# GPflow/GPflow

Hardware: AMD Instinct MI355X
Metric: svgp_elbo_steps_per_s (higher is better)
Workload: dtype f64; 1 GPU; SVGP RBF(ARD)+Gaussian ELBO, N=1e+06 M=2048 D=8 P=1 whitened, 8192 minibatch rows per GPU per step (BASELINE metric config Cm); global_batch=8192

## Files before the change

### gpflow_amd/csrc/gemm.hip

```cpp
#include "gpk_internal.h"
#include <mutex>
#include <stdlib.h>
#include <algorithm>
#include <type_traits>

namespace {

constexpr int BK = kGemmBK;
constexpr int LDSS = kGemmLDSS;
constexpr int GROUP_N = kGemmGroupN;

template <int BM, int BN, int WGM, int WGN>
struct TileCfg {
  static constexpr int WM = BM / WGM, WN = BN / WGN;
  static constexpr int TM = WM / 16, TN = WN / 16;
  static constexpr int A_CH = BM * (BK / 2) / 256;
  static constexpr int B_CH = BN * (BK / 2) / 256;
  static constexpr size_t LDS_BYTES = 2 * (size_t)(BM + BN) * LDSS * sizeof(double);
};

__device__ __forceinline__ void tile_decode(int nl, int gx, int gy, int compact, int& tile_m, int& tile_n) {
  tile_m = 0; tile_n = 0;
  if (compact) {
    int g = 0;
// ... 34 lines not shown
  const int xcd = lin & 7, local = lin >> 3;
  const int q = total >> 3, r = total & 7;
  int nl = xcd * q + (xcd < r ? xcd : r) + local;
  if (b_tri == 1 && gx > GROUP_N) nl = lin;
  tile_decode(nl, gx, gy, compact, tile_m, tile_n);
}

__device__ __forceinline__ d2 load2(const double* __restrict__ base, long ld, int row, int nrows,
                                    int k, int ke, bool vec_ok) {
  d2 v = {0.0, 0.0};
  if (row < nrows && k < ke) {
    const double* ptr = base + (long)row * ld + k;
    if (vec_ok && k + 1 < ke) {
      v = *reinterpret_cast<const d2*>(ptr);
    } else {
      v.x = ptr[0];
      if (k + 1 < ke) v.y = ptr[1];
    }
  }
  return v;
}

template <int BM, int BN, int WGM, int WGN>
__global__ __launch_bounds__(256, 2) void gemm_nt_kernel(GemmArgs p, int gx, int gy, int total, int compact) {
  using Cfg = TileCfg<BM, BN, WGM, WGN>;
  constexpr int WM = Cfg::WM, WN = Cfg::WN, TM = Cfg::TM, TN = Cfg::TN;
  constexpr int A_CH = Cfg::A_CH, B_CH = Cfg::B_CH;
  extern __shared__ __attribute__((aligned(16))) double smem[];
  if (p.sig_ptr && threadIdx.x == 0 && blockIdx.x == 0 && blockIdx.y == 0)
    __hip_atomic_store(p.sig_ptr, p.sig_val, __ATOMIC_RELAXED, __HIP_MEMORY_SCOPE_SYSTEM);

  const int tid = threadIdx.x, lane = tid & 63, wave = tid >> 6;
  const int wm = wave / WGN, wn = wave % WGN;
  const int bz = p.k_off_step ? (int)gridDim.y - 1 - (int)blockIdx.y : (int)blockIdx.y;

  int tile_m, tile_n;
  if (BM == 64 && BN == 64 && p.tail_first1 > 0) {
    int tm, tn;
    tile_decode(p.tail_first1 - 1 + ((int)blockIdx.x >> 2), gx, gy, compact, tm, tn);
    tile_m = 2 * tm + (((int)blockIdx.x >> 1) & 1);
    tile_n = 2 * tn + ((int)blockIdx.x & 1);
  } else if (p.tile_snake) {
    const int r = (int)blockIdx.x >> 8, c = (int)blockIdx.x & 255, R = (int)gridDim.x >> 8;
    const int rr = (r & 1) ? R - 1 - (r >> 1) : (r >> 1);
    if (p.tile_snake == 2) {
      const int xcd = c & 7, s = c >> 3, rpx = gy >> 3;
      const int q = rr * 32 + (((r ^ bz) & 1) ? 31 - s : s);
      tile_n = q / rpx;
      tile_m = xcd * rpx + (q - tile_n * rpx);
    } else {
      const int nl = rr * 256 + ((r & 1) ? 255 - c : c);
      if (nl >= total) return;
      tile_n = nl / gy;
      tile_m = nl - tile_n * gy;
    }
  } else {
    tile_order(blockIdx.x, p.b_tri, gx, gy, total, compact, tile_m, tile_n);
  }
  const int m0 = tile_m * BM, n0 = tile_n * BN;
  if (p.c_lower && n0 > m0 + BM - 1) return;
  if (m0 >= p.m || n0 >= p.n) return;

  const double* __restrict__ A = p.A + (long)bz * p.strideA;
  const double* __restrict__ B = p.B + (long)bz * p.strideB;

  int kb = 0, ke = p.k;
  const int koff = bz * p.k_off_step;
  if (p.b_tri && (n0 + BN < p.n ? n0 + BN : p.n) <= p.b_tri_rows) {
    if (p.b_tri == 1) {
      int f = n0 + p.b_tri_off - koff;
      kb = (f > 0 ? f : 0) & ~(BK - 1);
    } else {
      int l = n0 + BN + p.b_tri_off - koff;
      ke = l < p.k ? l : p.k;
    }
  }
  if (p.a_tri == 1) {
    int f = m0 - koff;
    f = (f > 0 ? f : 0) & ~(BK - 1);
    kb = kb > f ? kb : f;
  } else if (p.a_tri == 2) {
// ... 158 lines not shown
        } else {
          if ((lane & 15) == 0) smem[wn * BM + (row - m0)] = s;
        }
      }
    if constexpr (WN < 64) {
      constexpr int WPS = 64 / WN;
      __syncthreads();
      if (wn % WPS == 0 && (lane & 15) == 0) {
#pragma unroll
        for (int i = 0; i < TM; ++i)
#pragma unroll
          for (int r = 0; r < 4; ++r) {
            const int row = row_base + i * 16 + 4 * r;
            double s = smem[wn * BM + (row - m0)];
#pragma unroll
            for (int u = 1; u < WPS; ++u) s += smem[(wn + u) * BM + (row - m0)];
            if (row < p.m) part[(long)(tile_n * (BN / 64) + (wn * WN) / 64) * p.part_ld + row] = s;
          }
      }
    }
  }
}


__global__ __launch_bounds__(256, 2) void gemm_nt_pre64(GemmArgs p, int gx, int gy, int total, int compact) {
  constexpr int BM = 64, BN = 64, MAXS = 8;
  constexpr int BUF = (BM + BN) * LDSS;
  extern __shared__ __attribute__((aligned(16))) double smem[];
  if (p.sig_ptr && threadIdx.x == 0 && blockIdx.x == 0 && blockIdx.y == 0)
    __hip_atomic_store(p.sig_ptr, p.sig_val, __ATOMIC_RELAXED, __HIP_MEMORY_SCOPE_SYSTEM);

  const int tid = threadIdx.x, lane = tid & 63, wave = tid >> 6;
  const int bz = blockIdx.y;
  int tile_m, tile_n;
  tile_order(blockIdx.x, 0, gx, gy, total, compact, tile_m, tile_n);
  const int m0 = tile_m * BM, n0 = tile_n * BN;
  if (p.c_lower && n0 > m0 + BM - 1) return;
  if (m0 >= p.m || n0 >= p.n) return;
  const double* __restrict__ A = p.A + (long)bz * p.strideA;
  const double* __restrict__ B = p.B + (long)bz * p.strideB;
  double* __restrict__ C = p.C + (long)bz * p.strideC;
  const int nkt = p.k / BK;

  d2 ra[MAXS][2], rb[MAXS][2];
  const double* pa[2];
  const double* pb[2];
// ... 581 lines not shown
      }
      return GPK_E_UNSUPPORTED;
    default: break;
  }
  constexpr int FAST = (int)kGemmFastLds, WHOLE = 160 * 1024;
  if (p.queue) {
    unsigned qbase = 0;
    GPK_TRY(queue_slot(p.queue_fetches, &b.queue, &qbase));
    b.queue_base = (int)qbase;
    return launch_tiled<gemm_nt_fast<0, false, true>, FAST>(s, grid, p.lds_bytes, b, p, p.total);
  }
  int rc = GPK_E_UNSUPPORTED;
  switch (4 * p.epi + 2 * p.pair + p.sp) {
    case 0: rc = launch_tiled<gemm_nt_fast<0, false, false, 0>, WHOLE>(s, grid, p.lds_bytes, b, p, p.total); break;
    case 2: rc = launch_tiled<gemm_nt_fast<0, true, false, 0>, FAST>(s, grid, p.lds_bytes, b, p, p.total); break;
    case 4: rc = launch_tiled<gemm_nt_fast<1, false, false, 0>, WHOLE>(s, grid, p.lds_bytes, b, p, p.total); break;
    case 5: rc = launch_tiled<gemm_nt_fast<1, false, false, 1>, WHOLE>(s, grid, p.lds_bytes, b, p, p.total); break;
    case 6: rc = launch_tiled<gemm_nt_fast<1, true, false, 0>, FAST>(s, grid, p.lds_bytes, b, p, p.total); break;
    case 7: rc = launch_tiled<gemm_nt_fast<1, true, false, 1>, FAST>(s, grid, p.lds_bytes, b, p, p.total); break;
  }
  if (rc || p.tail_tiles == 0) return rc;
  GemmArgs t = a;
  t.tail_first1 = p.tail_first1;
  return launch_generic<64, 64, 4, 1>(s, dim3(p.tail_grid_x, 1, 1), t, p, (int)p.tail_grid_x);
}

}

int gpk_gemm_tiles_n(int n) { return gpk_cdiv(n, 128); }
bool gpk_gemm_takes_latency_kernel(const GemmArgs& a) { return make_gemm_plan(a).kernel == GemmKernel::small; }
bool gpk_gemm_fuses_row_stats(const GemmArgs& a) {
  const GemmPlan p = make_gemm_plan(a);
  return p.kernel == GemmKernel::fast && p.sp;
}

namespace {
struct ProfRec { hipEvent_t e0, e1; double flops; int kind; };
bool g_prof_on = false;
ProfRec* g_prof = nullptr;
int g_prof_n = 0, g_prof_cap = 0;

double algorithmic_flops(const GemmArgs& a) {
  const double m = a.m, n = a.n, k = a.k;
  double outs = m * n;
  if (a.c_lower) outs = (m >= n) ? n * (n + 1) / 2 + (m - n) * n : m * (m + 1) / 2;
  double kk = k;
  if (a.b_tri) {
// ... 151 lines not shown
```

### gpflow_amd/csrc/gemm_plan.h

```cpp
#pragma once
#include <stddef.h>
#include <stdint.h>
#include "gpk_tune.h"

struct GemmArgs {
  const double* A; long lda; long strideA;
  const double* B; long ldb; long strideB;
  double* C; long ldc; long strideC;
  int m, n, k;
  double alpha, beta;
  int c_lower;
  int b_tri;
  int a_tri;
  int b_tri_off;
  int b_tri_rows;
  int k_off_step;
  int epi;
  int sq_cols;
  double* part; long part_ld; long stridePart;
  double* C2; long ldc2; long strideC2; int c2_cols;
  double* stat_sumsq; double* stat_mv; const double* stat_V; int stat_P;
  int batch;
  int stagger_first;
  int stagger_ticks;
// ... 42 lines not shown
  switch (t) {
    case GemmTile::t128x128: return {128, 128, 2, 2};
    case GemmTile::t128x64: return {128, 64, 2, 2};
    case GemmTile::t64x128_1x4: return {64, 128, 1, 4};
    case GemmTile::t64x128_2x2: return {64, 128, 2, 2};
    case GemmTile::t64x64: return {64, 64, 4, 1};
    default: return {32, 64, 2, 2};
  }
}
constexpr size_t gemm_tile_lds(int bm, int bn) { return 2 * (size_t)(bm + bn) * kGemmLDSS * sizeof(double); }

struct GemmPlan {
  GemmKernel kernel = GemmKernel::none;
  GemmTile tile = GemmTile::t128x128;
  int epi = 0, pair = 0, queue = 0, sp = 0;
  int kind = 0;
  int gx = 0, gy = 0, total = 0, compact = 0;
  int ldk = 0;
  unsigned grid_x = 0, grid_y = 0, grid_z = 0;
  unsigned threads = 0;
  size_t lds_bytes = 0;
  int tile_snake = 0, stagger_first = 0, stagger_ticks = 0, pair_k_align = 0, tail_first1 = 0;
  int tail_tiles = 0;
  unsigned tail_grid_x = 0;
  unsigned queue_wgs = 0, queue_fetches = 0;
};

static inline int gemm_cdiv(int a, int b) { return (a + b - 1) / b; }
static inline int gemm_nbatch(const GemmArgs& a) { return a.batch > 0 ? a.batch : 1; }

static inline int gemm_lower_tiles(int gx, int gy) {
  int total = 0;
  for (int first = 0; first < gx; first += kGemmGroupN) {
    const int gsz = (gx - first) < kGemmGroupN ? (gx - first) : kGemmGroupN;
    const int avail = gy - first;
    if (avail <= 0) break;
    const int tr = avail < gsz ? avail : gsz;
    total += tr * (tr + 1) / 2 + (avail > gsz ? (avail - gsz) * gsz : 0);
  }
  return total;
}

static inline bool gemm_rows_16b(const GemmArgs& a) {
  if ((a.lda & 1) || (a.ldb & 1) || (a.strideA & 1) || (a.strideB & 1)) return false;
  return !((reinterpret_cast<uintptr_t>(a.A) & 15) || (reinterpret_cast<uintptr_t>(a.B) & 15));
}

// ... 144 lines not shown
                          : 0;
  }
  if (EPI == 0 && a.max_wgs > 0 && nwg < (unsigned)total && nb == 1) {
    const int kb = GPK_TUNE(CAP_EXCL_LDS_KB, 84);
    if (kb > 0 && kb <= 160 && (size_t)kb * 1024 > kGemmFastLds) p.lds_bytes = (size_t)kb * 1024;
  }
  if (EPI == 0 && tail_tiles == 0 && a.max_wgs == 0 &&
      ((a.k_off_step && GPK_TUNE(KSPLIT_QUEUE, 1)) || (a.tile_queue && (long)total * nb > 512))) {
    p.queue = 1;
    p.stagger_ticks = 0;
    const long all = (long)total * nb;
    const long qw = a.stagger_first > 0 ? 2L * a.stagger_first : GPK_TUNE(QUEUE_WGS, 512);
    p.queue_wgs = (unsigned)(all < qw ? all : qw);
    p.queue_fetches = (unsigned)all + p.queue_wgs;
    p.lds_bytes = kGemmFastLds;
    p.grid_x = p.queue_wgs; p.grid_y = 1;
    return;
  }
  p.grid_x = nwg;
  if (tail_tiles > 0) {
    p.tail_tiles = tail_tiles;
    p.tail_first1 = total_all - tail_tiles + 1;
    p.tail_grid_x = (unsigned)(4 * tail_tiles);
  }
}

static inline GemmPlan make_gemm_plan(const GemmArgs& a) {
  GemmPlan p;
  p.tile_snake = a.tile_snake; p.stagger_first = a.stagger_first; p.stagger_ticks = a.stagger_ticks;
  p.pair_k_align = a.pair_k_align;
  if (a.m <= 0 || a.n <= 0) return p;
  const auto unsupported = [&p]() { p.kernel = GemmKernel::unsupported; return p; };
  if (a.stat_sumsq && !gemm_row_stats_fusable(a)) return unsupported();
  const long tiles = (long)gemm_cdiv(a.m, 128) * gemm_cdiv(a.n, 128) * gemm_nbatch(a);
  if (a.tile64 && a.epi == 0) {
    if (GPK_TUNE(REST_PRE64, 1) && gemm_pre64_ok(a)) gemm_plan_pre64(a, p);
    else gemm_plan_generic(a, p, GemmTile::t64x64);
    return p;
  }
  if (!a.no_small && gemm_small_ok(a)) {
    gemm_plan_small(a, p);
    return p;
  }
  if (a.epi == 1 && a.beta != 0.0 && a.C && !gemm_fast_ok(a)) return unsupported();
  GemmTile tile = GemmTile::t128x128;
  if (a.epi == 0 && a.k >= GPK_TUNE(HALF_TILE_KMIN, 1024) && a.m > 64 && a.n > 64 && (a.max_wgs == 0 || a.max_wgs >= tiles) &&
      (a.c_lower ? tiles / 2 : tiles) < GPK_TUNE(HALF_TILE_BELOW, 300)) {
    tile = GemmTile::t64x128_1x4;
  } else if (gemm_proj_small_tiles(a)) {
    p.tile_snake = GPK_TUNE(PROJ_SNAKE, 1);
    if (gemm_cdiv(a.n, 64) != 2 * gemm_cdiv(a.n, 128)) tile = GemmTile::t64x128_2x2;
    else tile = gemm_proj_pairs(a) < GPK_TUNE(PROJ_TILE32_BELOW, 100) ? GemmTile::t32x64 : GemmTile::t64x64;
  } else if (gemm_fast_ok(a) && (a.epi == 1 || (a.n > 64 && (tiles >= 24 || a.m <= 64)))) {
    gemm_plan_fast(a, p);
    return p;
  } else if (a.epi == 1) {
    tile = GemmTile::t128x128;
  } else if (a.n <= 64) {
    tile = GemmTile::t128x64;
  } else if (tiles < 192 && a.m > 64) {
    tile = GemmTile::t64x128_1x4;
  }
  gemm_plan_generic(a, p, tile);
  return p;
}
```

### gpflow_amd/csrc/group_solve.hip

```cpp
#include "gpk_internal.h"
#include <algorithm>

namespace {


struct GroupSolveArgs {
  const double* E; long lde;
  double* Eo; long ldeo;
  const double* L; long ldl;
  const double* X;
  int rows, nb;
  long strideE, strideEo, strideL, strideX;
  int j0, j1;
};

__global__ __launch_bounds__(512) void group_solve_kernel(GroupSolveArgs p) {
  constexpr int LDK = 130, NBK = 128;
  {
    const long b = blockIdx.y;
    p.E += b * p.strideE; p.Eo += b * p.strideEo; p.L += b * p.strideL; p.X += b * p.strideX;
  }
  extern __shared__ __attribute__((aligned(16))) double smem[];
  const int tid = threadIdx.x, lane = tid & 63;
  const int wave = __builtin_amdgcn_readfirstlane(tid >> 6);
  const int r = lane & 15, g = lane >> 4;
  double* As = smem;
  double* Bs = smem + 16 * LDK;
  for (int m0 = blockIdx.x * 16; m0 < p.rows; m0 += gridDim.x * 16) {
  if (m0 != (int)blockIdx.x * 16) __syncthreads();
  int rowi[4];
#pragma unroll
  for (int e = 0; e < 4; ++e) {
    const int rr = m0 + g + 4 * e;
    rowi[e] = rr < p.rows ? rr : p.rows - 1;
  }
  const int colw = wave * 16 + r;
// ... 47 lines not shown
    __syncthreads();
    put_a(sj);
#pragma unroll
    for (int jp = 1; jp < 4; ++jp) {
      if (jp <= j || jp >= p.nb) continue;
      if (jp > j + 1) __syncthreads();
      stage_b(p.L + (long)jp * NBK * p.ldl + (long)j * NBK, p.ldl);
      __builtin_amdgcn_s_waitcnt(0x0070);
      __syncthreads();
      d4 u0, u1 = {0.0, 0.0, 0.0, 0.0};
#pragma unroll
      for (int e = 0; e < 4; ++e) u0[e] = -1.0 * c[jp][e];
      product(u0, u1);
#pragma unroll
      for (int e = 0; e < 4; ++e) c[jp][e] = -1.0 * (u0[e] + u1[e]);
    }
  }
  }
}


constexpr int GS2_LDK = 130;
constexpr int GS2_QK = 32, GS2_RING = 3;
constexpr size_t GS2_LDS = (size_t)(32 * GS2_LDK + GS2_RING * 128 * GS2_QK) * sizeof(double);

template <int DPW, int NMAX>
__device__ __forceinline__ void gs2_wait_vm(int n) {
  if constexpr (NMAX > 0) {
    if (n >= NMAX) {
      constexpr int c = NMAX * DPW;
      static_assert(c < 64, "vmcnt");
      __builtin_amdgcn_s_waitcnt(0x0F70 | (c & 15) | ((c >> 4) << 14));
      return;
    }
    gs2_wait_vm<DPW, NMAX - 1>(n);
  } else {
    __builtin_amdgcn_s_waitcnt(0x0F70);
  }
}

__global__ __launch_bounds__(512) void group_solve2_kernel(GroupSolveArgs p) {
  constexpr int LDK = GS2_LDK, NBK = 128, QK = GS2_QK, RING = GS2_RING;
  constexpr int AHEAD = RING - 1;
  constexpr int NQ = NBK / QK;
  constexpr int QELEMS = 128 * QK;
  constexpr int CH = QK / 2;
  constexpr int DROWS = 64 / CH;
  constexpr int DPW = (128 / DROWS) / 8;
  static_assert(QK == 32, "stage width: the chunk swizzle below");
  {
    const long b = blockIdx.y;
    p.E += b * p.strideE; p.Eo += b * p.strideEo; p.L += b * p.strideL; p.X += b * p.strideX;
  }
  extern __shared__ __attribute__((aligned(16))) double smem[];
  const int tid = threadIdx.x, lane = tid & 63;
  const int wave = __builtin_amdgcn_readfirstlane(tid >> 6);
  const int r = lane & 15, g = lane >> 4;
  double* As = smem;
  double* Bq = smem + 32 * LDK;
  const int nb = p.nb, j0 = p.j0, j1 = p.j1;
  int nprod = 0;
  for (int j = j0; j < j1; ++j) nprod += nb - j;
  const int nstages = NQ * nprod;
  auto swz = [](int row) -> int { return row & 15; };
  const int drow = lane / CH, dslot = lane % CH;
  const int drow0 = wave * DPW * DROWS + drow;
  int issue = 0, pj = j0, pjp = j0, pq = 0;
  auto issue_stage = [&]() {
    if (issue < nstages) {
      const bool isx = pjp == pj;
      const double* src = (isx ? p.X + (long)pj * NBK * NBK : p.L + (long)pjp * NBK * p.ldl + (long)pj * NBK) + pq * QK;
      const unsigned ld = isx ? (unsigned)NBK : (unsigned)p.ldl;
      double* dst = Bq + (issue % RING) * QELEMS;
#pragma unroll
      for (int i = 0; i < DPW; ++i) {
        const int rb = wave * DPW + i;
        const int row = drow0 + i * DROWS;
        const double* gsrc = src + ((unsigned)row * ld + (unsigned)((dslot ^ swz(row)) << 1));
        __builtin_amdgcn_global_load_lds((const __attribute__((address_space(1))) void*)gsrc,
                                         (__attribute__((address_space(3))) void*)(dst + rb * 128), 16, 0, 0);
      }
      if (++pq == NQ) {
        pq = 0;
        if (pjp + 1 < nb) ++pjp;
        else { ++pj; pjp = pj; }
      }
    }
    ++issue;
  };
  const int brow = (wave * 16 + r) * QK + (g & 1);
  const int bsw = swz(r), bgh = g >> 1;
  const double* ap = As + r * LDK + g;
  for (int m0 = blockIdx.x * 32; m0 < p.rows; m0 += gridDim.x * 32) {
    if (m0 != (int)blockIdx.x * 32) __syncthreads();
    issue = 0; pj = j0; pjp = j0; pq = 0;
    int cs = 0;
#pragma unroll
    for (int a = 0; a < AHEAD; ++a) issue_stage();
    const int colw = wave * 16 + r;
    int rowi[2][4];
#pragma unroll
    for (int t = 0; t < 2; ++t)
#pragma unroll
      for (int e = 0; e < 4; ++e) {
        const int rr = m0 + 16 * t + g + 4 * e;
        rowi[t][e] = rr < p.rows ? rr : p.rows - 1;
      }
    d4 c[2][4];
#pragma unroll
    for (int t = 0; t < 2; ++t)
#pragma unroll
      for (int jb = 0; jb < 4; ++jb) {
        if (jb >= j0 && jb < nb) {
#pragma unroll
          for (int e = 0; e < 4; ++e) c[t][jb][e] = p.E[(long)rowi[t][e] * p.lde + jb * NBK + colw];
        }
      }
    auto put_a = [&](const d4& v0, const d4& v1) {
#pragma unroll
      for (int e = 0; e < 4; ++e) {
        As[(g + 4 * e) * LDK + colw] = v0[e];
        As[(16 + g + 4 * e) * LDK + colw] = v1[e];
      }
    };
    auto stage = [&](int q, d4 (&acc)[2][2], bool a_changed) {
      {
        const int behind = nstages - 1 - cs < AHEAD - 1 ? nstages - 1 - cs : AHEAD - 1;
        gs2_wait_vm<DPW, AHEAD - 1>(behind);
      }
      asm volatile("" ::: "memory");
      if (a_changed) {
        __builtin_amdgcn_s_waitcnt(0xC07F);
        __builtin_amdgcn_s_barrier();
      }
      issue_stage();
      const double* bq = Bq + (cs % RING) * QELEMS + brow;
      double fb[2], fa0[2], fa1[2];
      auto frag = [&](int kk, int f) {
        fb[f] = bq[((2 * kk + bgh) ^ bsw) << 1];
        fa0[f] = ap[q * QK + kk * 4];
        fa1[f] = ap[16 * LDK + q * QK + kk * 4];
      };
      frag(0, 0);
#pragma unroll
      for (int kk = 0; kk < QK / 4; ++kk) {
        if (kk + 1 < QK / 4) frag(kk + 1, (kk + 1) & 1);
        acc[0][kk & 1] = __builtin_amdgcn_mfma_f64_16x16x4f64(fa0[kk & 1], fb[kk & 1], acc[0][kk & 1], 0, 0, 0);
        acc[1][kk & 1] = __builtin_amdgcn_mfma_f64_16x16x4f64(fa1[kk & 1], fb[kk & 1], acc[1][kk & 1], 0, 0, 0);
        __builtin_amdgcn_sched_group_barrier(0x008, 1, 0);
        if (kk + 1 < QK / 4) __builtin_amdgcn_sched_group_barrier(0x100, 3, 0);
        __builtin_amdgcn_sched_group_barrier(0x008, 1, 0);
      }
      ++cs;
    };
#pragma unroll
    for (int j = 0; j < 4; ++j) {
      if (j < j0) continue;
      if (j >= j1) break;
      if (j > j0) __syncthreads();
      put_a(c[0][j], c[1][j]);
      d4 acc[2][2];
#pragma unroll
      for (int t = 0; t < 2; ++t) { acc[t][0] = (d4){0.0, 0.0, 0.0, 0.0}; acc[t][1] = (d4){0.0, 0.0, 0.0, 0.0}; }
#pragma unroll
      for (int q = 0; q < NQ; ++q) stage(q, acc, q == 0);
      d4 sj[2];
#pragma unroll
      for (int t = 0; t < 2; ++t) {
#pragma unroll
        for (int e = 0; e < 4; ++e) sj[t][e] = 1.0 * (acc[t][0][e] + acc[t][1][e]);
#pragma unroll
        for (int e = 0; e < 4; ++e) {
          const int rr = m0 + 16 * t + g + 4 * e;
          if (rr < p.rows) p.Eo[(long)rr * p.ldeo + j * NBK + colw] = sj[t][e];
        }
      }
      if (j + 1 >= nb) break;
      __syncthreads();
      put_a(sj[0], sj[1]);
#pragma unroll
      for (int jp = 1; jp < 4; ++jp) {
        if (jp <= j || jp >= nb) continue;
#pragma unroll
        for (int t = 0; t < 2; ++t) {
#pragma unroll
          for (int e = 0; e < 4; ++e) acc[t][0][e] = -1.0 * c[t][jp][e];
          acc[t][1] = (d4){0.0, 0.0, 0.0, 0.0};
        }
#pragma unroll
        for (int q = 0; q < NQ; ++q) stage(q, acc, q == 0 && jp == j + 1);
#pragma unroll
        for (int t = 0; t < 2; ++t)
#pragma unroll
          for (int e = 0; e < 4; ++e) c[t][jp][e] = -1.0 * (acc[t][0][e] + acc[t][1][e]);
      }
    }
#pragma unroll
    for (int jp = 1; jp < 4; ++jp) {
      if (jp < j1 || jp >= nb) continue;
#pragma unroll
      for (int t = 0; t < 2; ++t)
#pragma unroll
        for (int e = 0; e < 4; ++e) {
          const int rr = m0 + 16 * t + g + 4 * e;
          if (rr < p.rows) p.Eo[(long)rr * p.ldeo + jp * NBK + colw] = c[t][jp][e];
        }
    }
  }
}

struct GroupSolveChoice { bool pipelined; unsigned wgs; };
GroupSolveChoice group_solve_choice(int rows, int batch, int max_wgs, bool partial) {
  const long slivers16 = (long)gpk_cdiv(rows, 16) * batch;
  GroupSolveChoice c;
  c.pipelined = GPK_TUNE(GROUP_SOLVE_V2, 1) && (partial || slivers16 > GPK_TUNE(GROUP_SOLVE_V2_MIN_SLIVERS, 256));
  c.wgs = (unsigned)gpk_cdiv(rows, c.pipelined ? 32 : 16);
  if (max_wgs > 0 && c.wgs * (unsigned)batch > (unsigned)max_wgs) c.wgs = (unsigned)std::max(1, max_wgs / batch);
  return c;
}

}

bool gpk_group_solve_takes_parts() { return group_solve_choice(1, 1, 0, true).pipelined; }

int gpk_launch_group_solve(hipStream_t s, const double* E, long lde, double* Eo, long ldeo, int rows, const double* Lgg, long ldl,
                           const double* X, int nb, int batch, long strideE, long strideEo, long strideL, long strideX, int max_wgs,
                           int j0, int j1) {
  if (rows <= 0) return 0;
  if (j1 < 0) j1 = nb;
  if (j0 < 0 || j0 >= j1 || j1 > nb) return GPK_E_ARG;
  const bool partial = j0 > 0 || j1 < nb;
  if (partial && (E != Eo || lde != ldeo || strideE != strideEo || !gpk_group_solve_takes_parts())) return GPK_E_UNSUPPORTED;
  if (batch < 1) batch = 1;
  if (!E || !Eo || !Lgg || !X || nb < 1 || nb > 4) return GPK_E_ARG;
  if ((ldl & 1) || (reinterpret_cast<uintptr_t>(Lgg) & 15) || (reinterpret_cast<uintptr_t>(X) & 15)) return GPK_E_UNSUPPORTED;
  if (batch > 1 && ((strideL & 1) || (strideX & 1))) return GPK_E_UNSUPPORTED;
  constexpr size_t LDS = (size_t)(16 + 128) * 130 * sizeof(double);
  static const hipError_t attr = hipFuncSetAttribute(reinterpret_cast<const void*>(group_solve_kernel),
                                                     hipFuncAttributeMaxDynamicSharedMemorySize, (int)LDS);
  GPK_HIP(attr);
  GroupSolveArgs a{};
  a.E = E; a.lde = lde; a.Eo = Eo; a.ldeo = ldeo; a.L = Lgg; a.ldl = ldl; a.X = X; a.rows = rows; a.nb = nb;
  a.strideE = strideE; a.strideEo = strideEo; a.strideL = strideL; a.strideX = strideX;
  a.j0 = j0; a.j1 = j1;
  const GroupSolveChoice c = group_solve_choice(rows, batch, max_wgs, partial);
  const dim3 grid(c.wgs, (unsigned)batch);
  if (c.pipelined) {
    static const hipError_t attr2 = hipFuncSetAttribute(reinterpret_cast<const void*>(group_solve2_kernel),
                                                        hipFuncAttributeMaxDynamicSharedMemorySize, (int)GS2_LDS);
    GPK_HIP(attr2);
    hipLaunchKernelGGL(group_solve2_kernel, grid, dim3(512), GS2_LDS, s, a);
  } else {
    hipLaunchKernelGGL(group_solve_kernel, grid, dim3(512), LDS, s, a);
  }
  GPK_LAUNCH_CHECK();
  return 0;
}
```

### gpflow_amd/csrc/potrf.hip

```cpp
#include "gpk_internal.h"
#include "potrf_plan.h"
#include <algorithm>
#include <mutex>
#include <vector>

namespace {
constexpr int NB = kPotrfNB;
constexpr int NBO = kPotrfNBO;
}

extern "C" const char* gpk_version(void) {
#ifdef GPK_EXPERIMENTAL
  return "gpk 0.4 (gfx950, fp64 MFMA) [A/B build: environment tunables enabled]";
#else
  return "gpk 0.4 (gfx950, fp64 MFMA)";
#endif
}

extern "C" size_t gpk_invd_elems(int n, int batch) {
  return (size_t)(batch > 0 ? batch : 1) * gpk_cdiv(n, NB) * NB * NB;
}

namespace {
struct Aux {
// ... 602 lines not shown
                               nfull, 1);
      if (rc) return rc;
    }
    if (nfull < nblk) {
      const int j0 = nfull * NB;
      int rc = gpk_launch_leaf(s, Lb + (long)j0 * (ldl + 1), ldl, 0, n - j0, ib + (long)nfull * NB * NB,
                               0, nullptr, 0, 1, 1);
      if (rc) return rc;
    }
  }
  return 0;
}

extern "C" int gpk_trsm(void* stream, int trans, const double* L, long ldl, const double* invd,
                        int n, double* B, int m, long ldb, int batch, long strideL, long strideB) {
  if (n < 0 || m < 0) return GPK_E_ARG;
  if (n == 0 || m == 0) return 0;
  if (!L || !invd || !B) return GPK_E_ARG;
  hipStream_t s = (hipStream_t)stream;
  if (batch <= 0) batch = 1;
  const long strideInv = (long)gpk_cdiv(n, NB) * NB * NB;
  int rc;
  if (trans == 0) {
    for (int g0 = 0; g0 < n; g0 += NBO) {
      rc = solve_group_fwd(s, PotrfBulk{}, B, ldb, B, ldb, m, L, ldl, invd, strideInv, n, g0, std::min(g0 + NBO, n), batch,
                           strideB, strideB, strideL);
      if (rc) return rc;
    }
  } else {
    const int ng = gpk_cdiv(n, NBO);
    for (int g = ng - 1; g >= 0; --g) {
      rc = solve_group_bwd(s, B, ldb, m, L, ldl, invd, strideInv, g * NBO, std::min((g + 1) * NBO, n), batch, strideB,
                           strideL);
      if (rc) return rc;
    }
  }
  return 0;
}

extern "C" int gpk_transpose_factor(void* stream, const double* L, long ldl, const double* invd,
                                    int n, double* LT, long ldlt, double* invdT) {
  if (!L || !invd || !LT || !invdT || n < 0) return GPK_E_ARG;
  if (n == 0) return 0;
  int rc = gpk_transpose(stream, L, n, n, ldl, LT, ldlt, 1, 1, 0, 0);
  if (rc) return rc;
  const int nblk = gpk_cdiv(n, NB);
  return gpk_transpose(stream, invd, NB, NB, NB, invdT, NB, 0, nblk, (long)NB * NB, (long)NB * NB);
}
// ... 1 lines not shown
```

### gpflow_amd/csrc/potrf_plan.h

```cpp
#pragma once
#include <algorithm>
#include <vector>
#include "../../include/gpk.h"
#include "gpk_tune.h"

constexpr int kPotrfNB = GPK_NB;
constexpr int kPotrfNBO = 512;
constexpr int kMaxFlagPanels = 512;

struct PotrfShape {
  int n, extra, batch, tri;
};
struct PotrfDevice {
  int bulk_cus;
  bool flags_usable;
};

enum class PotrfStream : unsigned char { B_masked, Bs, X };

struct PotrfBulk {
  int cap = 0;
  int group_cap = 0;
  int kmin = 256;
  template <class Gemm>
  void apply(Gemm& g) const {
    if (cap > 0 && g.k >= kmin) g.max_wgs = cap;
  }
};

struct PotrfPanel {
  int c0, c1, c2, c3;
  bool narrow;
  bool x_group_end;
  int x_group_begin;
  int x_progressive_block;
  bool tail_zone;
  bool flag_candidate;
  PotrfStream rest_stream;
  bool rest_tile_queue;
  bool rest_tile64_candidate;
  bool rest_small_loop;
  bool rest_flag;
  bool rest_split_candidate;
};

struct PotrfPlan {
  int n = 0, extra = 0, batch = 1, tri = 0;
  bool single_leaf = false;
  bool large = false;
  int nbo = kPotrfNB;
  bool ride = false;
// ... 58 lines not shown
  const int nbo = pl.nbo = large ? (nbo_large >= NB ? nbo_large : NBO) : NB;
  const int narrow_tail = (nbo > NB) ? (GPK_TUNE(NARROW_TAIL, 4096) / NB) * NB : 0;
  int npanels = 0;
  for (int c = 0; c < n; ++npanels) c += (nbo > NB && n - c > narrow_tail) ? nbo : NB;
  pl.panels.reserve((size_t)npanels);
  for (int c = 0; c < n;) {
    PotrfPanel q{};
    q.c0 = c;
    c += (nbo > NB && n - c > narrow_tail) ? nbo : NB;
    q.c1 = std::min(c, n);
    pl.panels.push_back(q);
  }
  for (int p = 0; p < npanels; ++p) {
    pl.panels[p].c2 = (p + 1 < npanels) ? pl.panels[p + 1].c1 : n;
    pl.panels[p].c3 = (p + 2 < npanels) ? pl.panels[p + 2].c1 : n;
  }
  pl.ride = extra > 0 && extra <= 256;
  const int R = pl.R = pl.ride ? n + extra : n;
  const bool useX = pl.useX = extra > 0 && !pl.ride;
  pl.B = large ? PotrfStream::B_masked : PotrfStream::Bs;
  pl.X = large ? PotrfStream::B_masked : PotrfStream::X;
  if (!large) pl.bulk.cap = batch > 1 ? GPK_TUNE(EXTRA_MAX_WGS_BATCHED, 320) : GPK_TUNE(EXTRA_MAX_WGS, 224);
  if (!large) pl.bulk.group_cap = GPK_TUNE(GROUP_SOLVE_MAX_WGS, 0);
  if (!large) pl.bulk.kmin = GPK_TUNE(EXTRA_CAP_KMIN, 256);
  pl.chain_wgs = (!large && batch == 1) ? GPK_TUNE(CHAIN_MAX_WGS, 0) : 0;
  pl.nevents = 2 * npanels + 8;
  pl.use_flags = GPK_TUNE(CHAIN_FLAGS, 1) && (batch == 1 || GPK_TUNE(CHAIN_FLAGS_BATCHED, 1)) && dev.flags_usable;
  pl.gate_kernels = GPK_TUNE(GATE_KERNELS, 1) != 0;
  const int xgroup_small = batch > 1 ? GPK_TUNE(XGROUP_SMALL_BATCH, 256) : GPK_TUNE(XGROUP_SMALL, 384);
  const int xgroup_wide = (batch == 1 && n < 4096 && extra < GPK_TUNE(XGROUP_FEW_ROWS_BELOW, 6144)) ? GPK_TUNE(XGROUP_FEW_ROWS, 256) : GPK_TUNE(XGROUP, NBO);
  pl.xgroup = std::max(NB, ((n <= 1024 ? xgroup_small : xgroup_wide) / NB) * NB);
  pl.xgroup_first = std::max(NB, (GPK_TUNE(XGROUP_FIRST, 0) > 0 ? (GPK_TUNE(XGROUP_FIRST, 0) / NB) * NB : pl.xgroup));
  const int tail_zone_max_rows = n > 1024 ? GPK_TUNE(XTAIL_ZONE_MAX_ROWS, 6144) : GPK_TUNE(XTAIL_ZONE_MAX_ROWS_SMALL, 6144);
  pl.tail_zone = useX && !large && (nbo == NB) && (n >= 8 * NB) && (extra < tail_zone_max_rows);
  pl.rest_tiled = useX && !large && batch == 1 && extra >= GPK_TUNE(REST_TILED_MIN_ROWS, 3000);
  pl.rest_tiled_min_wgs = n > 1024 ? GPK_TUNE(REST_TILED_MIN_WGS, 30) : GPK_TUNE(REST_TILED_MIN_WGS_SMALL, 150);
  pl.rest_small_wgs = (useX && !large && batch == 1 && extra >= 6144) ? GPK_TUNE(REST_SMALL_WGS, 0) : 0;
  pl.rest_tile64 = GPK_TUNE(REST_TILE64, 1);
  pl.trail_queue = GPK_TUNE(TRAIL_QUEUE, 1);
  pl.bulk_cus = dev.bulk_cus;
  pl.prog_end = std::min(pl.xgroup_first, n);
  pl.prog_cap = GPK_TUNE(XFIRST_PART_WGS, 128);
  pl.progressive_candidate = useX && !large && nbo == NB && batch == 1 && GPK_TUNE(XFIRST_PROGRESSIVE, 1) && pl.prog_end >= 2 * NB &&
                             extra >= GPK_TUNE(XFIRST_PROGRESSIVE_MIN_ROWS, 6144);
  pl.late_panel = std::min(npanels - 1, GPK_TUNE(LATE_WORK_PANEL, 5));
  pl.rest_split_enabled = GPK_TUNE(REST_SPLIT, 1) && pl.use_flags;
// ... 19 lines not shown
```

Measured before the change: 559.1 steps/s.

## Cap workgroup counts for GEMM tails and group solves with mixed-size slivers

Splits the GEMM NT kernel into a tile device function and adds a persistent tail kernel that walks tail sub-tiles with a capped workgroup count, padding its LDS allocation to limit co-residency. The group triangular solve now mixes 48-row and 32-row slivers so that a workgroup cap still covers all rows in one round, and the Cholesky plan now applies that cap to the group solve when many extra rows are present. The aim is to keep these kernels within a bounded share of compute units so they can run alongside concurrent work. The trade-off is more per-workgroup serial work and larger register and LDS pressure in the 48-row path.

```diff
diff --git a/gpflow_amd/csrc/gemm.hip b/gpflow_amd/csrc/gemm.hip
--- a/gpflow_amd/csrc/gemm.hip
+++ b/gpflow_amd/csrc/gemm.hip
@@ -80,41 +80,14 @@
 }
 
 template <int BM, int BN, int WGM, int WGN>
-__global__ __launch_bounds__(256, 2) void gemm_nt_kernel(GemmArgs p, int gx, int gy, int total, int compact) {
+__device__ __forceinline__ void gemm_nt_tile(const GemmArgs& p, int tile_m, int tile_n, int bz) {
   using Cfg = TileCfg<BM, BN, WGM, WGN>;
   constexpr int WM = Cfg::WM, WN = Cfg::WN, TM = Cfg::TM, TN = Cfg::TN;
   constexpr int A_CH = Cfg::A_CH, B_CH = Cfg::B_CH;
   extern __shared__ __attribute__((aligned(16))) double smem[];
-  if (p.sig_ptr && threadIdx.x == 0 && blockIdx.x == 0 && blockIdx.y == 0)
-    __hip_atomic_store(p.sig_ptr, p.sig_val, __ATOMIC_RELAXED, __HIP_MEMORY_SCOPE_SYSTEM);
-
   const int tid = threadIdx.x, lane = tid & 63, wave = tid >> 6;
   const int wm = wave / WGN, wn = wave % WGN;
-  const int bz = p.k_off_step ? (int)gridDim.y - 1 - (int)blockIdx.y : (int)blockIdx.y;
-
-  int tile_m, tile_n;
-  if (BM == 64 && BN == 64 && p.tail_first1 > 0) {
-    int tm, tn;
-    tile_decode(p.tail_first1 - 1 + ((int)blockIdx.x >> 2), gx, gy, compact, tm, tn);
-    tile_m = 2 * tm + (((int)blockIdx.x >> 1) & 1);
-    tile_n = 2 * tn + ((int)blockIdx.x & 1);
-  } else if (p.tile_snake) {
-    const int r = (int)blockIdx.x >> 8, c = (int)blockIdx.x & 255, R = (int)gridDim.x >> 8;
-    const int rr = (r & 1) ? R - 1 - (r >> 1) : (r >> 1);
-    if (p.tile_snake == 2) {
-      const int xcd = c & 7, s = c >> 3, rpx = gy >> 3;
-      const int q = rr * 32 + (((r ^ bz) & 1) ? 31 - s : s);
-      tile_n = q / rpx;
-      tile_m = xcd * rpx + (q - tile_n * rpx);
-    } else {
-      const int nl = rr * 256 + ((r & 1) ? 255 - c : c);
-      if (nl >= total) return;
-      tile_n = nl / gy;
-      tile_m = nl - tile_n * gy;
-    }
-  } else {
-    tile_order(blockIdx.x, p.b_tri, gx, gy, total, compact, tile_m, tile_n);
-  }
+
   const int m0 = tile_m * BM, n0 = tile_n * BN;
   if (p.c_lower && n0 > m0 + BM - 1) return;
   if (m0 >= p.m || n0 >= p.n) return;
@@ -319,6 +292,48 @@
   }
 }
 
+template <int BM, int BN, int WGM, int WGN>
+__global__ __launch_bounds__(256, 2) void gemm_nt_kernel(GemmArgs p, int gx, int gy, int total, int compact) {
+  if (p.sig_ptr && threadIdx.x == 0 && blockIdx.x == 0 && blockIdx.y == 0)
+    __hip_atomic_store(p.sig_ptr, p.sig_val, __ATOMIC_RELAXED, __HIP_MEMORY_SCOPE_SYSTEM);
+  const int bz = p.k_off_step ? (int)gridDim.y - 1 - (int)blockIdx.y : (int)blockIdx.y;
+
+  int tile_m, tile_n;
+  if (p.tile_snake) {
+    const int r = (int)blockIdx.x >> 8, c = (int)blockIdx.x & 255, R = (int)gridDim.x >> 8;
+    const int rr = (r & 1) ? R - 1 - (r >> 1) : (r >> 1);
+    if (p.tile_snake == 2) {
+      const int xcd = c & 7, s = c >> 3, rpx = gy >> 3;
+      const int q = rr * 32 + (((r ^ bz) & 1) ? 31 - s : s);
+      tile_n = q / rpx;
+      tile_m = xcd * rpx + (q - tile_n * rpx);
+    } else {
+      const int nl = rr * 256 + ((r & 1) ? 255 - c : c);
+      if (nl >= total) return;
+      tile_n = nl / gy;
+      tile_m = nl - tile_n * gy;
+    }
+  } else {
+    tile_order(blockIdx.x, p.b_tri, gx, gy, total, compact, tile_m, tile_n);
+  }
+  gemm_nt_tile<BM, BN, WGM, WGN>(p, tile_m, tile_n, bz);
+}
+
+template <int HALVES>
+__global__ __launch_bounds__(256, 2) void gemm_nt_tail64(GemmArgs p, int gx, int gy, int parts, int compact) {
+  if (p.sig_ptr && threadIdx.x == 0 && blockIdx.x == 0 && blockIdx.y == 0)
+    __hip_atomic_store(p.sig_ptr, p.sig_val, __ATOMIC_RELAXED, __HIP_MEMORY_SCOPE_SYSTEM);
+  for (int q = (int)blockIdx.x; q < parts; q += (int)gridDim.x) {
+    int tm, tn;
+    if constexpr (HALVES) {
+      tile_decode(p.tail_first1 - 1 + (q >> 1), gx, gy, compact, tm, tn);
+      gemm_nt_tile<128, 64, 2, 2>(p, tm, 2 * tn + (q & 1), 0);
+    } else {
+      tile_decode(p.tail_first1 - 1 + (q >> 2), gx, gy, compact, tm, tn);
+      gemm_nt_tile<64, 64, 4, 1>(p, 2 * tm + ((q >> 1) & 1), 2 * tn + (q & 1), 0);
+    }
+  }
+}
 
 __global__ __launch_bounds__(256, 2) void gemm_nt_pre64(GemmArgs p, int gx, int gy, int total, int compact) {
   constexpr int BM = 64, BN = 64, MAXS = 8;
@@ -946,7 +961,8 @@
   if (rc || p.tail_tiles == 0) return rc;
   GemmArgs t = a;
   t.tail_first1 = p.tail_first1;
-  return launch_generic<64, 64, 4, 1>(s, dim3(p.tail_grid_x, 1, 1), t, p, (int)p.tail_grid_x);
+  if (p.tail_halves) return launch_tiled<gemm_nt_tail64<1>, WHOLE>(s, dim3(p.tail_wgs, 1, 1), p.tail_lds_bytes, t, p, 2 * p.tail_tiles);
+  return launch_tiled<gemm_nt_tail64<0>, WHOLE>(s, dim3(p.tail_wgs, 1, 1), p.tail_lds_bytes, t, p, (int)p.tail_grid_x);
 }
 
 }
diff --git a/gpflow_amd/csrc/gemm_plan.h b/gpflow_amd/csrc/gemm_plan.h
--- a/gpflow_amd/csrc/gemm_plan.h
+++ b/gpflow_amd/csrc/gemm_plan.h
@@ -88,7 +88,9 @@
   size_t lds_bytes = 0;
   int tile_snake = 0, stagger_first = 0, stagger_ticks = 0, pair_k_align = 0, tail_first1 = 0;
   int tail_tiles = 0;
-  unsigned tail_grid_x = 0;
+  unsigned tail_grid_x = 0, tail_wgs = 0;
+  int tail_halves = 0;
+  size_t tail_lds_bytes = 0;
   unsigned queue_wgs = 0, queue_fetches = 0;
 };
 
@@ -279,6 +281,17 @@
     p.tail_tiles = tail_tiles;
     p.tail_first1 = total_all - tail_tiles + 1;
     p.tail_grid_x = (unsigned)(4 * tail_tiles);
+    const size_t tile_lds = gemm_tile_lds(64, 64);
+    p.tail_wgs = p.tail_grid_x;
+    p.tail_lds_bytes = tile_lds;
+    if (GPK_TUNE(TAIL_WALK_CAPPED, 1)) {
+      p.tail_halves = GPK_TUNE(TAIL_HALVES, 0) && 4 * tail_tiles > a.max_wgs && 2 * tail_tiles <= a.max_wgs;
+      const unsigned parts = p.tail_halves ? 2u * (unsigned)tail_tiles : p.tail_grid_x;
+      const unsigned rounds = (parts + (unsigned)a.max_wgs - 1) / (unsigned)a.max_wgs;
+      p.tail_wgs = (parts + rounds - 1) / rounds;
+      const int kb = GPK_TUNE(CAP_EXCL_LDS_KB, 84);
+      if (kb > 0 && kb <= 160 && (size_t)kb * 1024 > tile_lds) p.tail_lds_bytes = (size_t)kb * 1024;
+    }
   }
 }
 
@@ -308,7 +321,7 @@
     p.tile_snake = GPK_TUNE(PROJ_SNAKE, 1);
     if (gemm_cdiv(a.n, 64) != 2 * gemm_cdiv(a.n, 128)) tile = GemmTile::t64x128_2x2;
     else tile = gemm_proj_pairs(a) < GPK_TUNE(PROJ_TILE32_BELOW, 100) ? GemmTile::t32x64 : GemmTile::t64x64;
-  } else if (gemm_fast_ok(a) && (a.epi == 1 || (a.n > 64 && (tiles >= 24 || a.m <= 64)))) {
+  } else if (gemm_fast_ok(a) && (a.epi == 1 || (a.n > 64 && (tiles >= 24 || a.m <= 64 || (a.max_wgs > 0 && a.max_wgs < tiles))))) {
     gemm_plan_fast(a, p);
     return p;
   } else if (a.epi == 1) {
diff --git a/gpflow_amd/csrc/group_solve.hip b/gpflow_amd/csrc/group_solve.hip
--- a/gpflow_amd/csrc/group_solve.hip
+++ b/gpflow_amd/csrc/group_solve.hip
@@ -1,4 +1,5 @@
 #include "gpk_internal.h"
+#include "potrf_plan.h"
 #include <algorithm>
 
 namespace {
@@ -12,6 +13,7 @@
   int rows, nb;
   long strideE, strideEo, strideL, strideX;
   int j0, j1;
+  int n48;
 };
 
 __global__ __launch_bounds__(512) void group_solve_kernel(GroupSolveArgs p) {
@@ -105,7 +107,8 @@
 
 constexpr int GS2_LDK = 130;
 constexpr int GS2_QK = 32, GS2_RING = 3;
-constexpr size_t GS2_LDS = (size_t)(32 * GS2_LDK + GS2_RING * 128 * GS2_QK) * sizeof(double);
+constexpr size_t gs2_lds(int T) { return (size_t)(16 * T * GS2_LDK + GS2_RING * 128 * GS2_QK) * sizeof(double); }
+static_assert(gs2_lds(3) <= 160 * 1024, "a 48-row sliver fits a compute unit's LDS");
 
 template <int DPW, int NMAX>
 __device__ __forceinline__ void gs2_wait_vm(int n) {
@@ -122,7 +125,8 @@
   }
 }
 
-__global__ __launch_bounds__(512) void group_solve2_kernel(GroupSolveArgs p) {
+template <int T>
+__device__ __forceinline__ void gs2_sliver(const GroupSolveArgs& p, int m0) {
   constexpr int LDK = GS2_LDK, NBK = 128, QK = GS2_QK, RING = GS2_RING;
   constexpr int AHEAD = RING - 1;
   constexpr int NQ = NBK / QK;
@@ -131,16 +135,12 @@
   constexpr int DROWS = 64 / CH;
   constexpr int DPW = (128 / DROWS) / 8;
   static_assert(QK == 32, "stage width: the chunk swizzle below");
-  {
-    const long b = blockIdx.y;
-    p.E += b * p.strideE; p.Eo += b * p.strideEo; p.L += b * p.strideL; p.X += b * p.strideX;
-  }
   extern __shared__ __attribute__((aligned(16))) double smem[];
   const int tid = threadIdx.x, lane = tid & 63;
   const int wave = __builtin_amdgcn_readfirstlane(tid >> 6);
   const int r = lane & 15, g = lane >> 4;
   double* As = smem;
-  double* Bq = smem + 32 * LDK;
+  double* Bq = smem + 16 * T * LDK;
   const int nb = p.nb, j0 = p.j0, j1 = p.j1;
   int nprod = 0;
   for (int j = j0; j < j1; ++j) nprod += nb - j;
@@ -174,131 +174,156 @@
   const int brow = (wave * 16 + r) * QK + (g & 1);
   const int bsw = swz(r), bgh = g >> 1;
   const double* ap = As + r * LDK + g;
-  for (int m0 = blockIdx.x * 32; m0 < p.rows; m0 += gridDim.x * 32) {
-    if (m0 != (int)blockIdx.x * 32) __syncthreads();
-    issue = 0; pj = j0; pjp = j0; pq = 0;
-    int cs = 0;
-#pragma unroll
-    for (int a = 0; a < AHEAD; ++a) issue_stage();
-    const int colw = wave * 16 + r;
-    int rowi[2][4];
-#pragma unroll
-    for (int t = 0; t < 2; ++t)
+  int cs = 0;
+#pragma unroll
+  for (int a = 0; a < AHEAD; ++a) issue_stage();
+  const int colw = wave * 16 + r;
+  int rowi[T][4];
+#pragma unroll
+  for (int t = 0; t < T; ++t)
+#pragma unroll
+    for (int e = 0; e < 4; ++e) {
+      const int rr = m0 + 16 * t + g + 4 * e;
+      rowi[t][e] = rr < p.rows ? rr : p.rows - 1;
+    }
+  d4 c[T][4];
+#pragma unroll
+  for (int t = 0; t < T; ++t)
+#pragma unroll
+    for (int jb = 0; jb < 4; ++jb) {
+      if (jb >= j0 && jb < nb) {
+#pragma unroll
+        for (int e = 0; e < 4; ++e) c[t][jb][e] = p.E[(long)rowi[t][e] * p.lde + jb * NBK + colw];
+      }
+    }
+  auto put_a = [&](const d4 (&v)[T]) {
+#pragma unroll
+    for (int t = 0; t < T; ++t)
+#pragma unroll
+      for (int e = 0; e < 4; ++e) As[(16 * t + g + 4 * e) * LDK + colw] = v[t][e];
+  };
+  auto stage = [&](int q, d4 (&acc)[T][2], bool a_changed) {
+    {
+      const int behind = nstages - 1 - cs < AHEAD - 1 ? nstages - 1 - cs : AHEAD - 1;
+      gs2_wait_vm<DPW, AHEAD - 1>(behind);
+    }
+    asm volatile("" ::: "memory");
+    if (a_changed) {
+      __builtin_amdgcn_s_waitcnt(0xC07F);
+      __builtin_amdgcn_s_barrier();
+    }
+    issue_stage();
+    const double* bq = Bq + (cs % RING) * QELEMS + brow;
+    double fb[2], fa[T][2];
+    auto frag = [&](int kk, int f) {
+      fb[f] = bq[((2 * kk + bgh) ^ bsw) << 1];
+#pragma unroll
+      for (int t = 0; t < T; ++t) fa[t][f] = ap[16 * t * LDK + q * QK + kk * 4];
+    };
+    frag(0, 0);
+#pragma unroll
+    for (int kk = 0; kk < QK / 4; ++kk) {
+      if (kk + 1 < QK / 4) frag(kk + 1, (kk + 1) & 1);
+#pragma unroll
+      for (int t = 0; t < T; ++t)
+        acc[t][kk & 1] = __builtin_amdgcn_mfma_f64_16x16x4f64(fa[t][kk & 1], fb[kk & 1], acc[t][kk & 1], 0, 0, 0);
+      __builtin_amdgcn_sched_group_barrier(0x008, 1, 0);
+      if (kk + 1 < QK / 4) __builtin_amdgcn_sched_group_barrier(0x100, T + 1, 0);
+      __builtin_amdgcn_sched_group_barrier(0x008, T - 1, 0);
+    }
+    ++cs;
+  };
+#pragma unroll
+  for (int j = 0; j < 4; ++j) {
+    if (j < j0) continue;
+    if (j >= j1) break;
+    if (j > j0) __syncthreads();
+    {
+      d4 ej[T];
+#pragma unroll
+      for (int t = 0; t < T; ++t) ej[t] = c[t][j];
+      put_a(ej);
+    }
+    d4 acc[T][2];
+#pragma unroll
+    for (int t = 0; t < T; ++t) { acc[t][0] = (d4){0.0, 0.0, 0.0, 0.0}; acc[t][1] = (d4){0.0, 0.0, 0.0, 0.0}; }
+#pragma unroll
+    for (int q = 0; q < NQ; ++q) stage(q, acc, q == 0);
+    d4 sj[T];
+#pragma unroll
+    for (int t = 0; t < T; ++t) {
+#pragma unroll
+      for (int e = 0; e < 4; ++e) sj[t][e] = 1.0 * (acc[t][0][e] + acc[t][1][e]);
 #pragma unroll
       for (int e = 0; e < 4; ++e) {
         const int rr = m0 + 16 * t + g + 4 * e;
-        rowi[t][e] = rr < p.rows ? rr : p.rows - 1;
-      }
-    d4 c[2][4];
-#pragma unroll
-    for (int t = 0; t < 2; ++t)
-#pragma unroll
-      for (int jb = 0; jb < 4; ++jb) {
-        if (jb >= j0 && jb < nb) {
-#pragma unroll
-          for (int e = 0; e < 4; ++e) c[t][jb][e] = p.E[(long)rowi[t][e] * p.lde + jb * NBK + colw];
-        }
-      }
-    auto put_a = [&](const d4& v0, const d4& v1) {
+        if (rr < p.rows) p.Eo[(long)rr * p.ldeo + j * NBK + colw] = sj[t][e];
+      }
+    }
+    if (j + 1 >= nb) break;
+    __syncthreads();
+    put_a(sj);
+#pragma unroll
+    for (int jp = 1; jp < 4; ++jp) {
+      if (jp <= j || jp >= nb) continue;
+#pragma unroll
+      for (int t = 0; t < T; ++t) {
+#pragma unroll
+        for (int e = 0; e < 4; ++e) acc[t][0][e] = -1.0 * c[t][jp][e];
+        acc[t][1] = (d4){0.0, 0.0, 0.0, 0.0};
+      }
+#pragma unroll
+      for (int q = 0; q < NQ; ++q) stage(q, acc, q == 0 && jp == j + 1);
+#pragma unroll
+      for (int t = 0; t < T; ++t)
+#pragma unroll
+        for (int e = 0; e < 4; ++e) c[t][jp][e] = -1.0 * (acc[t][0][e] + acc[t][1][e]);
+    }
+  }
+#pragma unroll
+  for (int jp = 1; jp < 4; ++jp) {
+    if (jp < j1 || jp >= nb) continue;
+#pragma unroll
+    for (int t = 0; t < T; ++t)
 #pragma unroll
       for (int e = 0; e < 4; ++e) {
-        As[(g + 4 * e) * LDK + colw] = v0[e];
-        As[(16 + g + 4 * e) * LDK + colw] = v1[e];
-      }
-    };
-    auto stage = [&](int q, d4 (&acc)[2][2], bool a_changed) {
-      {
-        const int behind = nstages - 1 - cs < AHEAD - 1 ? nstages - 1 - cs : AHEAD - 1;
-        gs2_wait_vm<DPW, AHEAD - 1>(behind);
-      }
-      asm volatile("" ::: "memory");
-      if (a_changed) {
-        __builtin_amdgcn_s_waitcnt(0xC07F);
-        __builtin_amdgcn_s_barrier();
-      }
-      issue_stage();
-      const double* bq = Bq + (cs % RING) * QELEMS + brow;
-      double fb[2], fa0[2], fa1[2];
-      auto frag = [&](int kk, int f) {
-        fb[f] = bq[((2 * kk + bgh) ^ bsw) << 1];
-        fa0[f] = ap[q * QK + kk * 4];
-        fa1[f] = ap[16 * LDK + q * QK + kk * 4];
-      };
-      frag(0, 0);
-#pragma unroll
-      for (int kk = 0; kk < QK / 4; ++kk) {
-        if (kk + 1 < QK / 4) frag(kk + 1, (kk + 1) & 1);
-        acc[0][kk & 1] = __builtin_amdgcn_mfma_f64_16x16x4f64(fa0[kk & 1], fb[kk & 1], acc[0][kk & 1], 0, 0, 0);
-        acc[1][kk & 1] = __builtin_amdgcn_mfma_f64_16x16x4f64(fa1[kk & 1], fb[kk & 1], acc[1][kk & 1], 0, 0, 0);
-        __builtin_amdgcn_sched_group_barrier(0x008, 1, 0);
-        if (kk + 1 < QK / 4) __builtin_amdgcn_sched_group_barrier(0x100, 3, 0);
-        __builtin_amdgcn_sched_group_barrier(0x008, 1, 0);
-      }
-      ++cs;
-    };
-#pragma unroll
-    for (int j = 0; j < 4; ++j) {
-      if (j < j0) continue;
-      if (j >= j1) break;
-      if (j > j0) __syncthreads();
-      put_a(c[0][j], c[1][j]);
-      d4 acc[2][2];
-#pragma unroll
-      for (int t = 0; t < 2; ++t) { acc[t][0] = (d4){0.0, 0.0, 0.0, 0.0}; acc[t][1] = (d4){0.0, 0.0, 0.0, 0.0}; }
-#pragma unroll
-      for (int q = 0; q < NQ; ++q) stage(q, acc, q == 0);
-      d4 sj[2];
-#pragma unroll
-      for (int t = 0; t < 2; ++t) {
-#pragma unroll
-        for (int e = 0; e < 4; ++e) sj[t][e] = 1.0 * (acc[t][0][e] + acc[t][1][e]);
-#pragma unroll
-        for (int e = 0; e < 4; ++e) {
-          const int rr = m0 + 16 * t + g + 4 * e;
-          if (rr < p.rows) p.Eo[(long)rr * p.ldeo + j * NBK + colw] = sj[t][e];
-        }
-      }
-      if (j + 1 >= nb) break;
-      __syncthreads();
-      put_a(sj[0], sj[1]);
-#pragma unroll
-      for (int jp = 1; jp < 4; ++jp) {
-        if (jp <= j || jp >= nb) continue;
-#pragma unroll
-        for (int t = 0; t < 2; ++t) {
-#pragma unroll
-          for (int e = 0; e < 4; ++e) acc[t][0][e] = -1.0 * c[t][jp][e];
-          acc[t][1] = (d4){0.0, 0.0, 0.0, 0.0};
-        }
-#pragma unroll
-        for (int q = 0; q < NQ; ++q) stage(q, acc, q == 0 && jp == j + 1);
-#pragma unroll
-        for (int t = 0; t < 2; ++t)
-#pragma unroll
-          for (int e = 0; e < 4; ++e) c[t][jp][e] = -1.0 * (acc[t][0][e] + acc[t][1][e]);
-      }
-    }
-#pragma unroll
-    for (int jp = 1; jp < 4; ++jp) {
-      if (jp < j1 || jp >= nb) continue;
-#pragma unroll
-      for (int t = 0; t < 2; ++t)
-#pragma unroll
-        for (int e = 0; e < 4; ++e) {
-          const int rr = m0 + 16 * t + g + 4 * e;
-          if (rr < p.rows) p.Eo[(long)rr * p.ldeo + jp * NBK + colw] = c[t][jp][e];
-        }
-    }
-  }
-}
-
-struct GroupSolveChoice { bool pipelined; unsigned wgs; };
+        const int rr = m0 + 16 * t + g + 4 * e;
+        if (rr < p.rows) p.Eo[(long)rr * p.ldeo + jp * NBK + colw] = c[t][jp][e];
+      }
+  }
+}
+
+template <bool MIX>
+__global__ __launch_bounds__(512) void group_solve2_kernel(GroupSolveArgs p) {
+  {
+    const long b = blockIdx.y;
+    p.E += b * p.strideE; p.Eo += b * p.strideEo; p.L += b * p.strideL; p.X += b * p.strideX;
+  }
+  const int n48 = MIX ? p.n48 : 0;
+  const int nsl = n48 + (p.rows - 48 * n48 + 31) / 32;
+  for (int s = blockIdx.x; s < nsl; s += gridDim.x) {
+    if (s != (int)blockIdx.x) __syncthreads();
+    if (MIX && s < n48) gs2_sliver<3>(p, 48 * s);
+    else gs2_sliver<2>(p, 48 * n48 + 32 * (s - n48));
+  }
+}
+
+struct GroupSolveChoice { bool pipelined; unsigned wgs; int n48; };
 GroupSolveChoice group_solve_choice(int rows, int batch, int max_wgs, bool partial) {
   const long slivers16 = (long)gpk_cdiv(rows, 16) * batch;
   GroupSolveChoice c;
   c.pipelined = GPK_TUNE(GROUP_SOLVE_V2, 1) && (partial || slivers16 > GPK_TUNE(GROUP_SOLVE_V2_MIN_SLIVERS, 256));
+  c.n48 = 0;
   c.wgs = (unsigned)gpk_cdiv(rows, c.pipelined ? 32 : 16);
-  if (max_wgs > 0 && c.wgs * (unsigned)batch > (unsigned)max_wgs) c.wgs = (unsigned)std::max(1, max_wgs / batch);
+  if (max_wgs > 0 && c.wgs * (unsigned)batch > (unsigned)max_wgs) {
+    const int cap = std::max(1, max_wgs / batch);
+    c.wgs = (unsigned)cap;
+    if (c.pipelined && GPK_TUNE(GROUP_SOLVE_48, 1)) {
+      const GroupSliverMix mix = group_sliver_mix(rows, cap);
+      c.n48 = mix.n48;
+      if (mix.slivers() < cap) c.wgs = (unsigned)mix.slivers();
+    }
+  }
   return c;
 }
 
@@ -329,10 +354,18 @@
   const GroupSolveChoice c = group_solve_choice(rows, batch, max_wgs, partial);
   const dim3 grid(c.wgs, (unsigned)batch);
   if (c.pipelined) {
-    static const hipError_t attr2 = hipFuncSetAttribute(reinterpret_cast<const void*>(group_solve2_kernel),
-                                                        hipFuncAttributeMaxDynamicSharedMemorySize, (int)GS2_LDS);
-    GPK_HIP(attr2);
-    hipLaunchKernelGGL(group_solve2_kernel, grid, dim3(512), GS2_LDS, s, a);
+    if (c.n48 > 0) {
+      a.n48 = c.n48;
+      static const hipError_t attr3 = hipFuncSetAttribute(reinterpret_cast<const void*>(group_solve2_kernel<true>),
+                                                          hipFuncAttributeMaxDynamicSharedMemorySize, (int)gs2_lds(3));
+      GPK_HIP(attr3);
+      hipLaunchKernelGGL(group_solve2_kernel<true>, grid, dim3(512), gs2_lds(3), s, a);
+    } else {
+      static const hipError_t attr2 = hipFuncSetAttribute(reinterpret_cast<const void*>(group_solve2_kernel<false>),
+                                                          hipFuncAttributeMaxDynamicSharedMemorySize, (int)gs2_lds(2));
+      GPK_HIP(attr2);
+      hipLaunchKernelGGL(group_solve2_kernel<false>, grid, dim3(512), gs2_lds(2), s, a);
+    }
   } else {
     hipLaunchKernelGGL(group_solve_kernel, grid, dim3(512), LDS, s, a);
   }
diff --git a/gpflow_amd/csrc/potrf.hip b/gpflow_amd/csrc/potrf.hip
--- a/gpflow_amd/csrc/potrf.hip
+++ b/gpflow_amd/csrc/potrf.hip
@@ -648,8 +648,10 @@
   const long strideInv = (long)gpk_cdiv(n, NB) * NB * NB;
   int rc;
   if (trans == 0) {
+    PotrfBulk bulk{};
+    bulk.group_cap = GPK_TUNE(TRSM_GROUP_MAX_WGS, 0);
     for (int g0 = 0; g0 < n; g0 += NBO) {
-      rc = solve_group_fwd(s, PotrfBulk{}, B, ldb, B, ldb, m, L, ldl, invd, strideInv, n, g0, std::min(g0 + NBO, n), batch,
+      rc = solve_group_fwd(s, bulk, B, ldb, B, ldb, m, L, ldl, invd, strideInv, n, g0, std::min(g0 + NBO, n), batch,
                            strideB, strideB, strideL);
       if (rc) return rc;
     }
diff --git a/gpflow_amd/csrc/potrf_plan.h b/gpflow_amd/csrc/potrf_plan.h
--- a/gpflow_amd/csrc/potrf_plan.h
+++ b/gpflow_amd/csrc/potrf_plan.h
@@ -27,6 +27,19 @@
     if (cap > 0 && g.k >= kmin) g.max_wgs = cap;
   }
 };
+
+struct GroupSliverMix {
+  int n48, n32;
+  int slivers() const { return n48 + n32; }
+};
+static inline GroupSliverMix group_sliver_mix(int rows, int cap) {
+  GroupSliverMix m{0, rows > 0 ? (rows + 31) / 32 : 0};
+  if (cap <= 0 || m.n32 <= cap || rows > 48L * cap) return m;
+  m.n48 = (rows - 32 * cap + 15) / 16;
+  const int left = rows - 48 * m.n48;
+  m.n32 = left > 0 ? (left + 31) / 32 : 0;
+  return m;
+}
 
 struct PotrfPanel {
   int c0, c1, c2, c3;
@@ -131,6 +144,9 @@
   pl.X = large ? PotrfStream::B_masked : PotrfStream::X;
   if (!large) pl.bulk.cap = batch > 1 ? GPK_TUNE(EXTRA_MAX_WGS_BATCHED, 320) : GPK_TUNE(EXTRA_MAX_WGS, 224);
   if (!large) pl.bulk.group_cap = GPK_TUNE(GROUP_SOLVE_MAX_WGS, 0);
+  if (!large && batch == 1 && extra >= GPK_TUNE(XFIRST_PROGRESSIVE_MIN_ROWS, 6144) && pl.bulk.group_cap == 0 &&
+      GPK_TUNE(GROUP_SOLVE_IN_CAP, 1))
+    pl.bulk.group_cap = pl.bulk.cap;
   if (!large) pl.bulk.kmin = GPK_TUNE(EXTRA_CAP_KMIN, 256);
   pl.chain_wgs = (!large && batch == 1) ? GPK_TUNE(CHAIN_MAX_WGS, 0) : 0;
   pl.nevents = 2 * npanels + 8;
```

Result: no change. 559.3 steps/s (median of 3 runs) (+0.0%).
